# Tealdragon204/nightcore-to-flac-analyzer

Hardware: AMD Instinct MI355X
Metric: 10 s windows/sec (CQT+onset, 22.05 kHz mono) at 1/2/4/8 GPUs; % HBM roofline (higher is better)
Workload: dtype f32

## Files before the change

nightcore-to-flac-analyzer_amd/csrc/cqt.hip:

```cpp
#include <algorithm>

#include "nc_block.h"
#include "nc_decim.h"
#include "nc_engine.h"
#include "nc_piptrack.h"

namespace nc {


struct ChromaPlan {
  const float* sig;
  const int64_t* chunk_off;
  const int64_t* chunk_len;
  int n_chunks;
  int64_t* oct_off;
  int64_t* oct_len;
  int* n_frames;
  int* n_tframes;
  int64_t* tf_base;
};

__device__ __forceinline__ int64_t chunk_oct_floats(int64_t L) {
  int64_t acc = 0;
  for (int i = 1; i < 7; ++i) {
// ... 211 lines not shown
      for (int w = 1; w < D3_NT / 64; ++w) m = fmaxf(m, wmax[w]);
      xmax[c + (base == 0 ? oo3 : oct_off[c * 7 + 3]) / 256 + blockIdx.x] = m;
    }
    d3_level1_inplace(e0, o0, 4 * m0 - 72, L1, h, out1);
    __syncthreads();
    d3_level(e0, o0, D3_N2, 2 * m0 - 24, L2, h, e0 + D3_U2, o0 + D3_U2, out2, 24, 2 * D3_T);
    __syncthreads();
    d3_level(e0 + D3_U2, o0 + D3_U2, D3_T, m0, L3, h, nullptr, nullptr, out3, 0, D3_T);
  }
}

constexpr int TP_WAVES = 16;
#ifndef TP_DYN_
#define TP_DYN_ 1
#endif
using TpTw = StagedTw<1024>;

struct PeakArgs {
  const float* sig;
  const int64_t* chunk_off;
  const int64_t* chunk_len;
  const int* n_tframes;
  const int64_t* tf_base;
  const int64_t* tp_base;
  int n_chunks;
  int64_t total_tframes;
  const float2* tw;
  const float* hann2048;
  float* peak_pitch;
  float* peak_mag;
  int* chunk_npk;
  const int* tf_skip;
  unsigned long long* span = nullptr;
};

__global__ __launch_bounds__(TP_WAVES * 64) void tuning_peaks_kernel(PeakArgs a) {
  const Span span_(a.span);
  extern __shared__ __attribute__((aligned(16))) char smem[];
  float2* sh_tw = reinterpret_cast<float2*>(smem);
  const int lane0 = threadIdx.x & 63, wave = __builtin_amdgcn_readfirstlane(threadIdx.x >> 6);
  float2* sh_hann = sh_tw + ((TpTw::size + 1) & ~1);
  float2* fftbuf = sh_hann + 1024 + wave * LdsSize<1024>::value;
  __shared__ int sh_next;
  if (threadIdx.x == 0) sh_next = 0;
  fill_staged_tw<1024>(sh_tw, a.tw, threadIdx.x, TP_WAVES * 64);
  for (int i = threadIdx.x; i < 1024; i += TP_WAVES * 64) sh_hann[i] = reinterpret_cast<const float2*>(a.hann2048)[i];
  __syncthreads();
  float2 hw[16];
  lds_read16_strided<0, 64 * 8>(hw, lds_addr(sh_hann + fft_in_lane(lane0)));
  const int64_t n_groups = (a.total_tframes + TP_WAVES - 1) / TP_WAVES;
  const int64_t gb = n_groups * blockIdx.x / gridDim.x, ge = n_groups * (blockIdx.x + 1) / gridDim.x;
  const int64_t f0 = gb * TP_WAVES, f1 = std::min<int64_t>(ge * TP_WAVES, a.total_tframes);
  WgFrameQueue fq(&sh_next, lane0);
  int c = -1, nt = 0, skip = 0;
  int64_t cb = 0, ce = -1, coff = 0, clen = 0, ctf = 0;
  for (int64_t grp = gb; TP_DYN_ || grp < ge; ++grp) {
    const int64_t gf = TP_DYN_ ? f0 + fq.take(lane0) : grp * TP_WAVES + wave;
    if (gf >= (TP_DYN_ ? f1 : a.total_tframes)) break;
    if (gf >= ce) {
      if (c < 0) {
        int lo = 0, hi = a.n_chunks - 1;
        while (lo < hi) {
          const int mid = (lo + hi + 1) >> 1;
          if (a.tp_base[mid] <= gf) lo = mid;
// ... 5 lines not shown
        while (c + 1 < a.n_chunks && a.tp_base[c + 1] <= gf);
      }
      c = uniform32(c);
      cb = uniform64(a.tp_base[c]);
      ce = uniform64(c + 1 < a.n_chunks ? a.tp_base[c + 1] : INT64_MAX);
      skip = uniform32(a.tf_skip ? a.tf_skip[c] : 0);
      nt = uniform32(a.n_tframes[c]);
      coff = uniform64(a.chunk_off[c]);
      clen = uniform64(a.chunk_len[c]);
      ctf = uniform64(a.tf_base[c]);
    }
    const int t = (int)(gf - cb) + skip;
    if (t >= nt) continue;
    int lane = lane0;
    asm volatile("" : "+v"(lane));
    const int jin = fft_in_lane(lane);
    const int64_t off = coff;
    const float* x = a.sig + off;
    const int64_t L = clen;
    const int64_t s0 = (int64_t)t * 512 - 1024;
    FftIn<1024> in;
    if (s0 >= 0 && s0 + 2048 <= L) {
      float2 xv[16];
      if ((off & 1) == 0) {
        const float2* x2 = reinterpret_cast<const float2*>(x + s0);
#pragma unroll
        for (int r = 0; r < 16; ++r) xv[r] = x2[jin + 64 * r];
      } else {
        const float* xs = x + s0;
#pragma unroll
        for (int r = 0; r < 16; ++r) xv[r] = make_float2(xs[2 * (jin + 64 * r)], xs[2 * (jin + 64 * r) + 1]);
      }
#pragma unroll
      for (int r = 0; r < 16; ++r) in[0][r] = make_float2(xv[r].x * hw[r].x, xv[r].y * hw[r].y);
    } else {
// ... 13 lines not shown
    float* S = reinterpret_cast<float*>(fftbuf);
    float pmax = 0.0f;
    rsplit_mirror<TpTw::split, false>(v, sh_tw, lane, [&](int k, float2 X, float2 XN) {
      const float p1 = fmaf(X.x, X.x, X.y * X.y), p2 = fmaf(XN.x, XN.x, XN.y * XN.y);
      S[k] = p1;
      pmax = fmaxf(pmax, fmaxf(p1, p2));
    });
    const float mx = __fsqrt_rn(wave_max_u(pmax));
#pragma unroll
    for (int q = 0; q < (kPipHi - kPipLo + 3 + 63) / 64; ++q) {
      const int k = kPipLo - 1 + 64 * q + lane;
      if (64 * (q + 1) <= kPipHi - kPipLo + 3 || k <= kPipHi + 1) S[k] = __fsqrt_rn(S[k]);
    }
    piptrack_append([&](int k) { return S[k]; }, mx, lane, &a.chunk_npk[c], a.peak_pitch + ctf * kPeakSlots,
                    a.peak_mag + ctf * kPeakSlots, reinterpret_cast<int*>(S + kPipKpk));
  }
}

constexpr int TS_NT = 1024;
__device__ __forceinline__ int tuning_bin(float r) {
  const double rd = (double)r;
  int j = (int)floor((rd + 0.5) * 100.0);
  j = max(0, min(99, j));
  auto edge = [](int i) { return i == 100 ? 0.5 : (double)i * (1.0 / 100.0) + (-0.5); };
  while (j > 0 && rd < edge(j)) --j;
  while (j < 99 && rd >= edge(j + 1)) ++j;
  return j;
}

__device__ __forceinline__ unsigned fkey(float f) {
// ... 251 lines not shown
  const unsigned lg = xcd_remap(blockIdx.x + gridDim.x * blockIdx.y, gridDim.x * gridDim.y);
  const int bx = (int)(lg % gridDim.x);
  const int c = (int)(lg / gridDim.x);
  const int tid = threadIdx.x, lane = tid & 63;
  const int wave = __builtin_amdgcn_readfirstlane(tid >> 6);
  const int oct = CM_LO + wave;
  const int T = a.n_frames[c], ti = a.tuning_idx[c], ex = a.oct_ex[c * 7 + oct];
  const int64_t yoff = a.oct_off[c * 7 + oct], Ly = a.oct_len[c * 7 + oct];
  const int t0 = bx * CH_FR;
  if (t0 >= T) return;
  const int nfr = min(CH_FR, T - t0);
  const uint4* bsrc = a.bfrag + (size_t)ti * (CM_KS * CM_SLICE);
  auto fetch_slice = [&](int ks) {
#pragma unroll
    for (int q = 0; q < CM_GQ; ++q) {
      int i = wave + CM_NW * q;
      if (i >= CM_NT * 2) i = wave;
      cm_dma16(bsrc + ks * CM_SLICE + i * 64 + lane, sB + (ks % CM_R) * CM_SLICE + i * 64);
    }
  };
  fetch_slice(0);

  const float* y = a.ws_oct + yoff;
  const int hop = 512 >> oct;
  const float sx = ldexpf(1.0f, ex);
  const int64_t s0 = (int64_t)t0 * hop - 512;
  const int S = (CH_FR - 1) * hop + kCqtNfft;
  const bool vec = s0 >= 0 && s0 + S <= Ly && (reinterpret_cast<uintptr_t>(y) & 15) == 0;
  const int kq = 8 * (lane >> 4);

  constexpr int aoffs[8] = {cm_aoff(0), cm_aoff(1), cm_aoff(2), cm_aoff(3), cm_aoff(4), cm_aoff(5), cm_aoff(6), cm_aoff(7)};
  const int pad = cm_pad(oct);
  const int img = cm_img(oct);
// ... 663 lines not shown
  pa.sig = sig;
  pa.chunk_off = chunk_off;
  pa.chunk_len = chunk_len;
  pa.n_tframes = w.n_tframes;
  pa.tf_base = w.tf_base;
  pa.tp_base = tp_base;
  pa.tf_skip = tf_skip;
  pa.n_chunks = n;
  pa.total_tframes = tfr - tf_skip_total;
  pa.tw = ctx.t.tw;
  pa.hann2048 = ctx.t.hann2048;
  pa.peak_pitch = w.peak_pitch;
  pa.peak_mag = w.peak_mag;
  pa.chunk_npk = w.chunk_npk;
  {
    const size_t lds = (((TpTw::size + 1) & ~1) + 1024 + (size_t)TP_WAVES * LdsSize<1024>::value) * sizeof(float2);
    const int64_t groups = (pa.total_tframes + TP_WAVES - 1) / TP_WAVES;
    const int grid = (int)std::max<int64_t>(1, std::min<int64_t>(groups, ctx.chroma_cus > 0 ? ctx.chroma_cus : ctx.num_cu));
    {
      KTimer kt_(ctx, "tuning_peaks", st);
      pa.span = kt_.span();
      hipLaunchKernelGGL(tuning_peaks_kernel, dim3(grid), dim3(TP_WAVES * 64), lds, st, pa);
    }
  }
  if (wait_event) NC_HIP(hipStreamWaitEvent(st, static_cast<hipEvent_t>(wait_event), 0));
  {
    KTimer kt_(ctx, "tuning_select", st);
    OctScale os;
    os.xmax = w.xmax;
    os.oct_off = w.oct_off;
    os.oct_len = w.oct_len;
// ... 57 lines not shown
```

nightcore-to-flac-analyzer_amd/csrc/stft.hip:

```cpp
#include <algorithm>

#include "nc_block.h"
#include "nc_engine.h"
#include "nc_piptrack.h"

#include "stft_args.h"

namespace nc {

constexpr int SM_HANN2 = 1024;
constexpr int SM_WAVES = 16;
constexpr int SM_THREADS = SM_WAVES * 64;
constexpr int SM_HALF = 528;
constexpr size_t SM_LDS_RESERVE = 150 * 1024;
#ifndef SM_NOEN_
#define SM_NOEN_ 0
#endif
#ifndef SM_SYNC_
#define SM_SYNC_ 0
#endif
#ifndef SM_DYN_
#define SM_DYN_ 1
#endif
using SmTw = StagedTw<1024>;

constexpr int kMelJ0 = 3, kMelJ1 = 14;
constexpr int kMelJ0w = 4, kMelJ1w = 17;
constexpr int kMelB = 7;

template <int J>
__device__ __forceinline__ void mel_unrolled(const float* pw, const float4* w4, int lo, int nj, int lane, float& acc) {
#pragma unroll
  for (int j0 = 0; j0 < J; j0 += kMelB) {
    float4 p[kMelB], w[kMelB];
#pragma unroll
    for (int j = 0; j < kMelB; ++j)
      if (j0 + j < J) {
        p[j] = *reinterpret_cast<const float4*>(pw + lo + 4 * (j0 + j));
        w[j] = w4[(j0 + j) * 64 + lane];
// ... 13 lines not shown
  }
  return lo;
}

__host__ __device__ __forceinline__ int al4(int n) { return (n + 3) & ~3; }

constexpr int SM_MT = 128;
__host__ __device__ __forceinline__ int mel_pack(int lo4, int nj4, int band) { return lo4 | (nj4 << 11) | (band << 16); }

size_t stft_mel_lds_bytes(int mel_j) {
  return (size_t)al4(SmTw::size) * sizeof(float2) + (size_t)mel_j * 64 * sizeof(float4) +
         (size_t)SM_HANN2 * sizeof(float2) + (size_t)SM_MT * sizeof(int) +
         (size_t)SM_WAVES * SM_HALF * sizeof(float2);
}

__device__ __forceinline__ int sm_j1(int l) {
  const int G = l >> 4, i = l & 15;
  return 4 * (8 * (G >> 1) + (i >> 1)) + (i & 1) + 2 * (G & 1);
}
__device__ __forceinline__ int sm_j2(int l) {
  return (l & 7) + 8 * (l >> 5) + 16 * ((l & 31) >> 3);
}
__host__ __device__ constexpr int sm_boff(int b) { return b == 0 ? 0 : b == 1 ? 136 : b == 2 ? 264 : 400; }
constexpr int kPipKpkHalf = 512;
static_assert(kPipKpkHalf >= kPipHi - kPipLo + 3 && kPipKpkHalf + (kPipHi - kPipLo + 1) <= 2 * SM_HALF,
              "piptrack half-slot layout");

#define NC_W_(v, o) "ds_write_b64 %[wb], %[" #v "] offset:" #o "\n\t"
#define NC_R_(d, b, o) "ds_read_b64 %[" #d "], %[" #b "] offset:" #o "\n\t"

__device__ __forceinline__ void sm_exchange1(const float2 (&v)[16], float2 (&u)[16], uint32_t wb, uint32_t rb) {
  nc_f2v i0 = {v[0].x, v[0].y}, i1 = {v[1].x, v[1].y}, i2 = {v[2].x, v[2].y}, i3 = {v[3].x, v[3].y};
  nc_f2v i4 = {v[4].x, v[4].y}, i5 = {v[5].x, v[5].y}, i6 = {v[6].x, v[6].y}, i7 = {v[7].x, v[7].y};
  nc_f2v i8 = {v[8].x, v[8].y}, i9 = {v[9].x, v[9].y}, i10 = {v[10].x, v[10].y}, i11 = {v[11].x, v[11].y};
  nc_f2v i12 = {v[12].x, v[12].y}, i13 = {v[13].x, v[13].y}, i14 = {v[14].x, v[14].y}, i15 = {v[15].x, v[15].y};
  nc_f2v d0, d1, d2, d3, d4, d5, d6, d7, d8, d9, d10, d11, d12, d13, d14, d15;
  unsigned long long sv;
  asm volatile(
      NC_W_(i0, 0) NC_W_(i1, 8) NC_W_(i2, 16) NC_W_(i3, 24) NC_W_(i4, 32) NC_W_(i5, 40) NC_W_(i6, 48) NC_W_(i7, 56)
      "s_mov_b64 %[sv], exec\n\t"
      "s_mov_b32 exec_hi, 0\n\t"
      NC_R_(d0, rb, 0) NC_R_(d1, rb, 264) NC_R_(d2, rb, 528) NC_R_(d3, rb, 792) NC_R_(d4, rb, 1056)
      NC_R_(d5, rb, 1320) NC_R_(d6, rb, 1584) NC_R_(d7, rb, 1848) NC_R_(d8, rb, 2112) NC_R_(d9, rb, 2376)
      NC_R_(d10, rb, 2640) NC_R_(d11, rb, 2904) NC_R_(d12, rb, 3168) NC_R_(d13, rb, 3432) NC_R_(d14, rb, 3696)
      NC_R_(d15, rb, 3960)
      "s_mov_b64 exec, %[sv]\n\t"
      NC_W_(i8, 0) NC_W_(i9, 8) NC_W_(i10, 16) NC_W_(i11, 24) NC_W_(i12, 32) NC_W_(i13, 40) NC_W_(i14, 48)
      NC_W_(i15, 56)
      "s_mov_b32 exec_lo, 0\n\t"
      NC_R_(d0, rb, 0) NC_R_(d1, rb, 264) NC_R_(d2, rb, 528) NC_R_(d3, rb, 792) NC_R_(d4, rb, 1056)
      NC_R_(d5, rb, 1320) NC_R_(d6, rb, 1584) NC_R_(d7, rb, 1848) NC_R_(d8, rb, 2112) NC_R_(d9, rb, 2376)
      NC_R_(d10, rb, 2640) NC_R_(d11, rb, 2904) NC_R_(d12, rb, 3168) NC_R_(d13, rb, 3432) NC_R_(d14, rb, 3696)
      NC_R_(d15, rb, 3960)
      "s_mov_b64 exec, %[sv]\n\t"
      "s_waitcnt lgkmcnt(0)"
      : [d0] "=&v"(d0), [d1] "=&v"(d1), [d2] "=&v"(d2), [d3] "=&v"(d3), [d4] "=&v"(d4), [d5] "=&v"(d5),
        [d6] "=&v"(d6), [d7] "=&v"(d7), [d8] "=&v"(d8), [d9] "=&v"(d9), [d10] "=&v"(d10), [d11] "=&v"(d11),
        [d12] "=&v"(d12), [d13] "=&v"(d13), [d14] "=&v"(d14), [d15] "=&v"(d15), [sv] "=&s"(sv)
      : [wb] "v"(wb), [rb] "v"(rb), [i0] "v"(i0), [i1] "v"(i1), [i2] "v"(i2), [i3] "v"(i3), [i4] "v"(i4),
        [i5] "v"(i5), [i6] "v"(i6), [i7] "v"(i7), [i8] "v"(i8), [i9] "v"(i9), [i10] "v"(i10), [i11] "v"(i11),
        [i12] "v"(i12), [i13] "v"(i13), [i14] "v"(i14), [i15] "v"(i15)
      : "memory");
  const nc_f2v d[16] = {d0, d1, d2, d3, d4, d5, d6, d7, d8, d9, d10, d11, d12, d13, d14, d15};
#pragma unroll
  for (int r = 0; r < 16; ++r) u[r] = make_float2(d[r].x, d[r].y);
}

__device__ __forceinline__ void sm_exchange2(const float2 (&v)[16], float2 (&o)[16], uint32_t wb, uint32_t r0,
                                             uint32_t r1, uint32_t r2, uint32_t r3) {
  nc_f2v i0 = {v[0].x, v[0].y}, i1 = {v[1].x, v[1].y}, i2 = {v[2].x, v[2].y}, i3 = {v[3].x, v[3].y};
  nc_f2v i4 = {v[4].x, v[4].y}, i5 = {v[5].x, v[5].y}, i6 = {v[6].x, v[6].y}, i7 = {v[7].x, v[7].y};
  nc_f2v i8 = {v[8].x, v[8].y}, i9 = {v[9].x, v[9].y}, i10 = {v[10].x, v[10].y}, i11 = {v[11].x, v[11].y};
  nc_f2v i12 = {v[12].x, v[12].y}, i13 = {v[13].x, v[13].y}, i14 = {v[14].x, v[14].y}, i15 = {v[15].x, v[15].y};
  nc_f2v d0, d1, d2, d3, d4, d5, d6, d7, d8, d9, d10, d11, d12, d13, d14, d15;
  asm volatile(
      NC_W_(i0, 0) NC_W_(i1, 128) NC_W_(i2, 256) NC_W_(i3, 384) NC_W_(i4, 512) NC_W_(i5, 640) NC_W_(i6, 768)
      NC_W_(i7, 896)
      NC_R_(d0, r0, 0) NC_R_(d1, r0, 1088) NC_R_(d2, r0, 2112) NC_R_(d3, r0, 3200)
      NC_R_(d4, r1, 0) NC_R_(d5, r1, 1088) NC_R_(d6, r1, 2112) NC_R_(d7, r1, 3200)
      NC_W_(i8, 0) NC_W_(i9, 128) NC_W_(i10, 256) NC_W_(i11, 384) NC_W_(i12, 512) NC_W_(i13, 640) NC_W_(i14, 768)
      NC_W_(i15, 896)
      NC_R_(d8, r2, 0) NC_R_(d9, r2, 1088) NC_R_(d10, r2, 2112) NC_R_(d11, r2, 3200)
      NC_R_(d12, r3, 0) NC_R_(d13, r3, 1088) NC_R_(d14, r3, 2112) NC_R_(d15, r3, 3200)
      "s_waitcnt lgkmcnt(0)"
      : [d0] "=&v"(d0), [d1] "=&v"(d1), [d2] "=&v"(d2), [d3] "=&v"(d3), [d4] "=&v"(d4), [d5] "=&v"(d5),
        [d6] "=&v"(d6), [d7] "=&v"(d7), [d8] "=&v"(d8), [d9] "=&v"(d9), [d10] "=&v"(d10), [d11] "=&v"(d11),
        [d12] "=&v"(d12), [d13] "=&v"(d13), [d14] "=&v"(d14), [d15] "=&v"(d15)
      : [wb] "v"(wb), [r0] "v"(r0), [r1] "v"(r1), [r2] "v"(r2), [r3] "v"(r3), [i0] "v"(i0), [i1] "v"(i1),
        [i2] "v"(i2), [i3] "v"(i3), [i4] "v"(i4), [i5] "v"(i5), [i6] "v"(i6), [i7] "v"(i7), [i8] "v"(i8),
        [i9] "v"(i9), [i10] "v"(i10), [i11] "v"(i11), [i12] "v"(i12), [i13] "v"(i13), [i14] "v"(i14),
        [i15] "v"(i15)
      : "memory");
  const nc_f2v d[16] = {d0, d1, d2, d3, d4, d5, d6, d7, d8, d9, d10, d11, d12, d13, d14, d15};
#pragma unroll
  for (int r = 0; r < 16; ++r) o[r] = make_float2(d[r].x, d[r].y);
}
#undef NC_W_
#undef NC_R_

template <bool H512, bool EN, int J0 = kMelJ0, int J1 = kMelJ1>
__global__ __launch_bounds__(SM_THREADS) void stft_mel_kernel(StftMelArgs a) {
  const Span span_(a.span);
  extern __shared__ __attribute__((aligned(16))) char smem[];
  float2* sh_tw = reinterpret_cast<float2*>(smem);
  float4* sh_w4 = reinterpret_cast<float4*>(sh_tw + al4(SmTw::size));
  const int lane0 = threadIdx.x & 63, wave = __builtin_amdgcn_readfirstlane(threadIdx.x >> 6);
  float2* sh_hann = reinterpret_cast<float2*>(sh_w4 + (a.mel_j0 + a.mel_j1) * 64);
  int* sh_mt = reinterpret_cast<int*>(sh_hann + SM_HANN2);
  float2* slot = reinterpret_cast<float2*>(sh_mt + SM_MT) + wave * SM_HALF;

  __shared__ int sh_next;
  if (threadIdx.x == 0) sh_next = 0;
  fill_staged_tw<1024>(sh_tw, a.tw, threadIdx.x, SM_THREADS);
// ... 39 lines not shown
      t0 = uniform64(a.frame_base && a.seq_t0 ? a.seq_t0[s] : 0);
      act = !a.active || a.active[s];
      L = uniform64(a.seq_len ? a.seq_len[s] : a.uniform_len);
      off = uniform64(a.seq_off[s]);
      wc = uniform32(a.win_chunk ? a.win_chunk[s] : -1);
    }
    if (!act) continue;
    const int64_t t = g - sb + t0;
    const float* x = a.sig + off;
    const int64_t s0 = t * a.hop - 1024;

    int lane = lane0;
    asm volatile("" : "+v"(lane));
    const int jin = sm_j1(lane);
    const float2* twl = sh_tw;
    const float* hann = a.hann2048;
    float2 in[16];
    double e = 0.0;
    const bool interior = s0 >= 0 && s0 + 2048 <= L;
    if (interior) {
      float2 xv[16];
      if ((off & 1) == 0) {
        const float2* x2 = reinterpret_cast<const float2*>(x + s0);
#pragma unroll
        for (int r = 0; r < 16; ++r) xv[r] = x2[jin + 64 * r];
      } else {
        const float* xs = x + s0;
#pragma unroll
        for (int r = 0; r < 16; ++r) xv[r] = make_float2(xs[2 * (jin + 64 * r)], xs[2 * (jin + 64 * r) + 1]);
      }
#pragma unroll
      for (int r = 0; r < 16; ++r) {
        const int n = jin + 64 * r;
        const float2 v = xv[r];
        const float2 h = hw[r];
        if (EN && r >= 8 && r < 12) {
          const bool in_hop = H512 || 2 * n - 1024 < a.hop;
          const double dx = in_hop ? (double)v.x : 0.0, dy = in_hop ? (double)v.y : 0.0;
          e = fma(dx, dx, e);
          e = fma(dy, dy, e);
        }
        in[r] = make_float2(v.x * h.x, v.y * h.y);
      }
    } else {
#pragma unroll
      for (int r = 0; r < 16; ++r) {
        const int n = jin + 64 * r;
        const int64_t i0 = s0 + 2 * n;
        const float x0 = (i0 >= 0 && i0 < L) ? x[i0] : 0.0f;
        const float x1 = (i0 + 1 >= 0 && i0 + 1 < L) ? x[i0 + 1] : 0.0f;
        if (EN && r >= 8 && r < 12) {
          const int q = 2 * n - 1024;
          if (q < a.hop) {
            e = fma((double)x0, (double)x0, e);
            e = fma((double)x1, (double)x1, e);
          }
        }
        in[r] = make_float2(x0 * hann[2 * n], x1 * hann[2 * n + 1]);
      }
    }
    if (EN) {
      e = wave_sum_u(e);
      if (lane == 0) a.frame_energy[g] = e;
    }
    DFT<16>::run(in);
    const int j2 = sm_j2(lane), k2 = j2 & 15;
    float2 v2[16];
    sm_exchange1(in, v2, lds_addr(slot + 8 * jin + (jin >> 2)), lds_addr(slot + (lane & 31)));
    {
      const uint32_t ta = lds_addr(twl + k2);
      tw_batch3<0, 16 * 8>(v2 + 1, ta);
      tw_batch3<3, 16 * 8>(v2 + 4, ta);
      tw_batch3<6, 16 * 8>(v2 + 7, ta);
      tw_batch3<9, 16 * 8>(v2 + 10, ta);
      tw_batch3<12, 16 * 8>(v2 + 13, ta);
    }
    DFT<16>::run(v2);
    float2 v[4][4];
    {
      const int b2 = j2 >> 4;
      float2 o[16];
      sm_exchange2(v2, o, lds_addr(slot + sm_boff(b2) + k2), lds_addr(slot + mirror_J(lane, 0)),
                   lds_addr(slot + mirror_J(lane, 1)), lds_addr(slot + (mirror_J(lane, 2) - 128)),
                   lds_addr(slot + (mirror_J(lane, 3) - 128)));
      static_for<4>([&](auto bc) {
        constexpr int b = decltype(bc)::value;
        float2 w[3];
        const uint32_t ta = lds_addr(twl + SmTw::s3 + mirror_J(lane, b));
        lds_read3<0, 2048, 4096>(w, ta, ta, ta);
        v[b][0] = o[4 * b];
#pragma unroll
        for (int r = 1; r < 4; ++r) v[b][r] = cmul(o[4 * b + r], w[r - 1]);
        DFT<4>::run(v[b]);
      });
    }
    float* pw = reinterpret_cast<float*>(slot);
    const bool pip = wc >= 0 && t < a.tp_frames;
    float pmax = 0.0f;
    if (pip) {
      rsplit_mirror<SmTw::split, false>(v, twl, lane, [&](int k, float2 X, float2 XN) {
        const float p1 = fmaf(X.x, X.x, X.y * X.y), p2 = fmaf(XN.x, XN.x, XN.y * XN.y);
        pw[k] = p1;
        pw[1024 - k] = p2;
        pmax = fmaxf(pmax, fmaxf(p1, p2));
      });
    } else {
      rsplit_mirror<SmTw::split, false>(v, twl, lane, [&](int k, float2 X, float2 XN) {
        pw[k] = fmaf(X.x, X.x, X.y * X.y);
        pw[1024 - k] = fmaf(XN.x, XN.x, XN.y * XN.y);
      });
    }
    float acc0 = 0.0f, acc1 = 0.0f;
    const int mt0 = sh_mt[lane], mt1 = sh_mt[64 + lane];
    mel_unrolled<J0>(pw, mw4, mt0 & 2047, (mt0 >> 11) & 31, lane, acc0);
    mel_unrolled<J1>(pw, mw4 + J0 * 64, mt1 & 2047, (mt1 >> 11) & 31, lane, acc1);
    const float db0 = db10_floor(acc0);
    const float db1 = db10_floor(acc1);
    float* row = a.sdb + g * 128;
    row[mt0 >> 16] = db0;
    row[mt1 >> 16] = db1;
    const float mx = wave_max_u(fmaxf(db0, db1));
    if (lane == 0) a.frame_max[g] = mx;
    if (pip) {
      const float pm = __fsqrt_rn(wave_max_u(pmax));
      constexpr int kPipQ = (kPipHi - kPipLo + 3 + 63) / 64;
      float pv[kPipQ];
#pragma unroll
      for (int q = 0; q < kPipQ; ++q) {
        const int k = kPipLo - 1 + 64 * q + lane;
        pv[q] = (64 * (q + 1) <= kPipHi - kPipLo + 3 || k <= kPipHi + 1) ? pw[k] : 0.0f;
      }
      asm volatile("" ::: "memory");
#pragma unroll
      for (int q = 0; q < kPipQ; ++q) {
        const int k = kPipLo - 1 + 64 * q + lane;
        if (64 * (q + 1) <= kPipHi - kPipLo + 3 || k <= kPipHi + 1) pw[k - (kPipLo - 1)] = __fsqrt_rn(pv[q]);
      }
      const int64_t base = uniform64(a.chunk_tf_base[wc]) * kPeakSlots;
      piptrack_append([&](int k) { return pw[k - (kPipLo - 1)]; }, pm, lane, &a.chunk_npk[wc], a.peak_pitch + base,
                      a.peak_mag + base, reinterpret_cast<int*>(pw + kPipKpkHalf));
    }
  }
}

int launch_stft_mel(Context& ctx, const StftMelArgs& args, hipStream_t st) {
  if (args.total_frames <= 0) return 0;
  StftMelArgs a = args;
  a.tw = ctx.t.tw;
  a.hann2048 = ctx.t.hann2048;
  a.mel_lo = ctx.t.mel_lo;
  a.mel_len = ctx.t.mel_len;
  a.mel_off = ctx.t.mel_off;
  a.mel_w = ctx.t.mel_w;
  a.mel_nnz = ctx.t.mel_nnz;
  a.mel_w4 = ctx.t.mel_w4;
// ... 58 lines not shown
```

Baseline: 486,600.

## Share the STFT frame FFT core with the tuning-peaks kernel and use compact LDS slots

Moves the hand-scheduled 1024-point frame FFT (custom lane mapping, inline-asm LDS exchanges, power and piptrack helpers) out of the STFT kernel into a shared header. The tuning-peaks kernel now uses this path by default in place of its generic Stockham FFT, with a smaller per-wave LDS slot, while still reserving the old LDS size. The chroma B-fragment prefetch also skips redundant duplicate DMA loads for waves past the slice count. The aim is fewer LDS operations and less FFT instruction overhead in the tuning kernel. The piptrack layout is now half-slot, and behaviour changes if the compact layout or the new lane mapping differ subtly from the old path.

```diff
diff --git a/nightcore-to-flac-analyzer_amd/csrc/cqt.hip b/nightcore-to-flac-analyzer_amd/csrc/cqt.hip
--- a/nightcore-to-flac-analyzer_amd/csrc/cqt.hip
+++ b/nightcore-to-flac-analyzer_amd/csrc/cqt.hip
@@ -3,7 +3,7 @@
 #include "nc_block.h"
 #include "nc_decim.h"
 #include "nc_engine.h"
-#include "nc_piptrack.h"
+#include "nc_frame_fft.h"
 
 namespace nc {
 
@@ -249,7 +249,15 @@
 #ifndef TP_DYN_
 #define TP_DYN_ 1
 #endif
-using TpTw = StagedTw<1024>;
+#ifndef TP_CORE_
+#define TP_CORE_ 1
+#endif
+using TpTw = FrameTw;
+constexpr int TP_SLOT = TP_CORE_ ? SM_HALF : LdsSize<1024>::value;
+constexpr size_t TP_LDS_BYTES = (((TpTw::size + 1) & ~1) + 1024 + (size_t)TP_WAVES * TP_SLOT) * sizeof(float2);
+#ifndef TP_LDS_RESERVE_
+#define TP_LDS_RESERVE_ ((((TpTw::size + 1) & ~1) + 1024 + TP_WAVES * LdsSize<1024>::value) * 8)
+#endif
 
 struct PeakArgs {
   const float* sig;
@@ -275,14 +283,14 @@
   float2* sh_tw = reinterpret_cast<float2*>(smem);
   const int lane0 = threadIdx.x & 63, wave = __builtin_amdgcn_readfirstlane(threadIdx.x >> 6);
   float2* sh_hann = sh_tw + ((TpTw::size + 1) & ~1);
-  float2* fftbuf = sh_hann + 1024 + wave * LdsSize<1024>::value;
+  float2* fftbuf = sh_hann + 1024 + wave * TP_SLOT;
   __shared__ int sh_next;
   if (threadIdx.x == 0) sh_next = 0;
   fill_staged_tw<1024>(sh_tw, a.tw, threadIdx.x, TP_WAVES * 64);
   for (int i = threadIdx.x; i < 1024; i += TP_WAVES * 64) sh_hann[i] = reinterpret_cast<const float2*>(a.hann2048)[i];
   __syncthreads();
   float2 hw[16];
-  lds_read16_strided<0, 64 * 8>(hw, lds_addr(sh_hann + fft_in_lane(lane0)));
+  lds_read16_strided<0, 64 * 8>(hw, lds_addr(sh_hann + (TP_CORE_ ? sm_j1(lane0) : fft_in_lane(lane0))));
   const int64_t n_groups = (a.total_tframes + TP_WAVES - 1) / TP_WAVES;
   const int64_t gb = n_groups * blockIdx.x / gridDim.x, ge = n_groups * (blockIdx.x + 1) / gridDim.x;
   const int64_t f0 = gb * TP_WAVES, f1 = std::min<int64_t>(ge * TP_WAVES, a.total_tframes);
@@ -318,11 +326,22 @@
     if (t >= nt) continue;
     int lane = lane0;
     asm volatile("" : "+v"(lane));
-    const int jin = fft_in_lane(lane);
+    const int jin = TP_CORE_ ? sm_j1(lane) : fft_in_lane(lane);
     const int64_t off = coff;
     const float* x = a.sig + off;
     const int64_t L = clen;
     const int64_t s0 = (int64_t)t * 512 - 1024;
+#if TP_CORE_
+    float2 in[16];
+    double e_ = 0.0;
+    frame_load_hann<false, true>(x, s0, L, (off & 1) != 0, 512, jin, hw, a.hann2048, in, e_);
+    float2 v[4][4];
+    frame_fft1024(in, fftbuf, sh_tw, lane, jin, v);
+    float* pw = reinterpret_cast<float*>(fftbuf);
+    float pmax = 0.0f;
+    frame_power<true, false>(v, sh_tw, lane, pw, pmax);
+    frame_piptrack(pw, pmax, lane, &a.chunk_npk[c], a.peak_pitch + ctf * kPeakSlots, a.peak_mag + ctf * kPeakSlots);
+#else
     FftIn<1024> in;
     if (s0 >= 0 && s0 + 2048 <= L) {
       float2 xv[16];
@@ -366,6 +385,7 @@
     }
     piptrack_append([&](int k) { return S[k]; }, mx, lane, &a.chunk_npk[c], a.peak_pitch + ctf * kPeakSlots,
                     a.peak_mag + ctf * kPeakSlots, reinterpret_cast<int*>(S + kPipKpk));
+#endif
   }
 }
 
@@ -647,9 +667,8 @@
   auto fetch_slice = [&](int ks) {
 #pragma unroll
     for (int q = 0; q < CM_GQ; ++q) {
-      int i = wave + CM_NW * q;
-      if (i >= CM_NT * 2) i = wave;
-      cm_dma16(bsrc + ks * CM_SLICE + i * 64 + lane, sB + (ks % CM_R) * CM_SLICE + i * 64);
+      const int i = wave + CM_NW * q;
+      if (i < CM_NT * 2) cm_dma16(bsrc + ks * CM_SLICE + i * 64 + lane, sB + (ks % CM_R) * CM_SLICE + i * 64);
     }
   };
   fetch_slice(0);
@@ -1343,7 +1362,7 @@
   pa.peak_mag = w.peak_mag;
   pa.chunk_npk = w.chunk_npk;
   {
-    const size_t lds = (((TpTw::size + 1) & ~1) + 1024 + (size_t)TP_WAVES * LdsSize<1024>::value) * sizeof(float2);
+    const size_t lds = std::max<size_t>(TP_LDS_BYTES, TP_LDS_RESERVE_);
     const int64_t groups = (pa.total_tframes + TP_WAVES - 1) / TP_WAVES;
     const int grid = (int)std::max<int64_t>(1, std::min<int64_t>(groups, ctx.chroma_cus > 0 ? ctx.chroma_cus : ctx.num_cu));
     {
diff --git a/nightcore-to-flac-analyzer_amd/csrc/nc_frame_fft.h b/nightcore-to-flac-analyzer_amd/csrc/nc_frame_fft.h
--- /dev/null
+++ b/nightcore-to-flac-analyzer_amd/csrc/nc_frame_fft.h
@@ -0,0 +1,204 @@
+#pragma once
+#include "nc_device.h"
+#include "nc_piptrack.h"
+
+namespace nc {
+
+using FrameTw = StagedTw<1024>;
+constexpr int SM_HALF = 528;
+
+__device__ __forceinline__ int sm_j1(int l) {
+  const int G = l >> 4, i = l & 15;
+  return 4 * (8 * (G >> 1) + (i >> 1)) + (i & 1) + 2 * (G & 1);
+}
+__device__ __forceinline__ int sm_j2(int l) {
+  return (l & 7) + 8 * (l >> 5) + 16 * ((l & 31) >> 3);
+}
+__host__ __device__ constexpr int sm_boff(int b) { return b == 0 ? 0 : b == 1 ? 136 : b == 2 ? 264 : 400; }
+constexpr int kPipKpkHalf = 512;
+static_assert(kPipKpkHalf >= kPipHi - kPipLo + 3 && kPipKpkHalf + (kPipHi - kPipLo + 1) <= 2 * SM_HALF,
+              "piptrack half-slot layout");
+
+#define NC_W_(v, o) "ds_write_b64 %[wb], %[" #v "] offset:" #o "\n\t"
+#define NC_R_(d, b, o) "ds_read_b64 %[" #d "], %[" #b "] offset:" #o "\n\t"
+
+__device__ __forceinline__ void sm_exchange1(const float2 (&v)[16], float2 (&u)[16], uint32_t wb, uint32_t rb) {
+  nc_f2v i0 = {v[0].x, v[0].y}, i1 = {v[1].x, v[1].y}, i2 = {v[2].x, v[2].y}, i3 = {v[3].x, v[3].y};
+  nc_f2v i4 = {v[4].x, v[4].y}, i5 = {v[5].x, v[5].y}, i6 = {v[6].x, v[6].y}, i7 = {v[7].x, v[7].y};
+  nc_f2v i8 = {v[8].x, v[8].y}, i9 = {v[9].x, v[9].y}, i10 = {v[10].x, v[10].y}, i11 = {v[11].x, v[11].y};
+  nc_f2v i12 = {v[12].x, v[12].y}, i13 = {v[13].x, v[13].y}, i14 = {v[14].x, v[14].y}, i15 = {v[15].x, v[15].y};
+  nc_f2v d0, d1, d2, d3, d4, d5, d6, d7, d8, d9, d10, d11, d12, d13, d14, d15;
+  unsigned long long sv;
+  asm volatile(
+      NC_W_(i0, 0) NC_W_(i1, 8) NC_W_(i2, 16) NC_W_(i3, 24) NC_W_(i4, 32) NC_W_(i5, 40) NC_W_(i6, 48) NC_W_(i7, 56)
+      "s_mov_b64 %[sv], exec\n\t"
+      "s_mov_b32 exec_hi, 0\n\t"
+      NC_R_(d0, rb, 0) NC_R_(d1, rb, 264) NC_R_(d2, rb, 528) NC_R_(d3, rb, 792) NC_R_(d4, rb, 1056)
+      NC_R_(d5, rb, 1320) NC_R_(d6, rb, 1584) NC_R_(d7, rb, 1848) NC_R_(d8, rb, 2112) NC_R_(d9, rb, 2376)
+      NC_R_(d10, rb, 2640) NC_R_(d11, rb, 2904) NC_R_(d12, rb, 3168) NC_R_(d13, rb, 3432) NC_R_(d14, rb, 3696)
+      NC_R_(d15, rb, 3960)
+      "s_mov_b64 exec, %[sv]\n\t"
+      NC_W_(i8, 0) NC_W_(i9, 8) NC_W_(i10, 16) NC_W_(i11, 24) NC_W_(i12, 32) NC_W_(i13, 40) NC_W_(i14, 48)
+      NC_W_(i15, 56)
+      "s_mov_b32 exec_lo, 0\n\t"
+      NC_R_(d0, rb, 0) NC_R_(d1, rb, 264) NC_R_(d2, rb, 528) NC_R_(d3, rb, 792) NC_R_(d4, rb, 1056)
+      NC_R_(d5, rb, 1320) NC_R_(d6, rb, 1584) NC_R_(d7, rb, 1848) NC_R_(d8, rb, 2112) NC_R_(d9, rb, 2376)
+      NC_R_(d10, rb, 2640) NC_R_(d11, rb, 2904) NC_R_(d12, rb, 3168) NC_R_(d13, rb, 3432) NC_R_(d14, rb, 3696)
+      NC_R_(d15, rb, 3960)
+      "s_mov_b64 exec, %[sv]\n\t"
+      "s_waitcnt lgkmcnt(0)"
+      : [d0] "=&v"(d0), [d1] "=&v"(d1), [d2] "=&v"(d2), [d3] "=&v"(d3), [d4] "=&v"(d4), [d5] "=&v"(d5),
+        [d6] "=&v"(d6), [d7] "=&v"(d7), [d8] "=&v"(d8), [d9] "=&v"(d9), [d10] "=&v"(d10), [d11] "=&v"(d11),
+        [d12] "=&v"(d12), [d13] "=&v"(d13), [d14] "=&v"(d14), [d15] "=&v"(d15), [sv] "=&s"(sv)
+      : [wb] "v"(wb), [rb] "v"(rb), [i0] "v"(i0), [i1] "v"(i1), [i2] "v"(i2), [i3] "v"(i3), [i4] "v"(i4),
+        [i5] "v"(i5), [i6] "v"(i6), [i7] "v"(i7), [i8] "v"(i8), [i9] "v"(i9), [i10] "v"(i10), [i11] "v"(i11),
+        [i12] "v"(i12), [i13] "v"(i13), [i14] "v"(i14), [i15] "v"(i15)
+      : "memory");
+  const nc_f2v d[16] = {d0, d1, d2, d3, d4, d5, d6, d7, d8, d9, d10, d11, d12, d13, d14, d15};
+#pragma unroll
+  for (int r = 0; r < 16; ++r) u[r] = make_float2(d[r].x, d[r].y);
+}
+
+__device__ __forceinline__ void sm_exchange2(const float2 (&v)[16], float2 (&o)[16], uint32_t wb, uint32_t r0,
+                                             uint32_t r1, uint32_t r2, uint32_t r3) {
+  nc_f2v i0 = {v[0].x, v[0].y}, i1 = {v[1].x, v[1].y}, i2 = {v[2].x, v[2].y}, i3 = {v[3].x, v[3].y};
+  nc_f2v i4 = {v[4].x, v[4].y}, i5 = {v[5].x, v[5].y}, i6 = {v[6].x, v[6].y}, i7 = {v[7].x, v[7].y};
+  nc_f2v i8 = {v[8].x, v[8].y}, i9 = {v[9].x, v[9].y}, i10 = {v[10].x, v[10].y}, i11 = {v[11].x, v[11].y};
+  nc_f2v i12 = {v[12].x, v[12].y}, i13 = {v[13].x, v[13].y}, i14 = {v[14].x, v[14].y}, i15 = {v[15].x, v[15].y};
+  nc_f2v d0, d1, d2, d3, d4, d5, d6, d7, d8, d9, d10, d11, d12, d13, d14, d15;
+  asm volatile(
+      NC_W_(i0, 0) NC_W_(i1, 128) NC_W_(i2, 256) NC_W_(i3, 384) NC_W_(i4, 512) NC_W_(i5, 640) NC_W_(i6, 768)
+      NC_W_(i7, 896)
+      NC_R_(d0, r0, 0) NC_R_(d1, r0, 1088) NC_R_(d2, r0, 2112) NC_R_(d3, r0, 3200)
+      NC_R_(d4, r1, 0) NC_R_(d5, r1, 1088) NC_R_(d6, r1, 2112) NC_R_(d7, r1, 3200)
+      NC_W_(i8, 0) NC_W_(i9, 128) NC_W_(i10, 256) NC_W_(i11, 384) NC_W_(i12, 512) NC_W_(i13, 640) NC_W_(i14, 768)
+      NC_W_(i15, 896)
+      NC_R_(d8, r2, 0) NC_R_(d9, r2, 1088) NC_R_(d10, r2, 2112) NC_R_(d11, r2, 3200)
+      NC_R_(d12, r3, 0) NC_R_(d13, r3, 1088) NC_R_(d14, r3, 2112) NC_R_(d15, r3, 3200)
+      "s_waitcnt lgkmcnt(0)"
+      : [d0] "=&v"(d0), [d1] "=&v"(d1), [d2] "=&v"(d2), [d3] "=&v"(d3), [d4] "=&v"(d4), [d5] "=&v"(d5),
+        [d6] "=&v"(d6), [d7] "=&v"(d7), [d8] "=&v"(d8), [d9] "=&v"(d9), [d10] "=&v"(d10), [d11] "=&v"(d11),
+        [d12] "=&v"(d12), [d13] "=&v"(d13), [d14] "=&v"(d14), [d15] "=&v"(d15)
+      : [wb] "v"(wb), [r0] "v"(r0), [r1] "v"(r1), [r2] "v"(r2), [r3] "v"(r3), [i0] "v"(i0), [i1] "v"(i1),
+        [i2] "v"(i2), [i3] "v"(i3), [i4] "v"(i4), [i5] "v"(i5), [i6] "v"(i6), [i7] "v"(i7), [i8] "v"(i8),
+        [i9] "v"(i9), [i10] "v"(i10), [i11] "v"(i11), [i12] "v"(i12), [i13] "v"(i13), [i14] "v"(i14),
+        [i15] "v"(i15)
+      : "memory");
+  const nc_f2v d[16] = {d0, d1, d2, d3, d4, d5, d6, d7, d8, d9, d10, d11, d12, d13, d14, d15};
+#pragma unroll
+  for (int r = 0; r < 16; ++r) o[r] = make_float2(d[r].x, d[r].y);
+}
+#undef NC_W_
+#undef NC_R_
+
+template <bool EN, bool H512>
+__device__ __forceinline__ void frame_load_hann(const float* x, int64_t s0, int64_t L, bool odd, int hop, int jin,
+                                                const float2 (&hw)[16], const float* hann, float2 (&in)[16],
+                                                double& e) {
+  const bool interior = s0 >= 0 && s0 + 2048 <= L;
+  if (interior) {
+    float2 xv[16];
+    if (!odd) {
+      const float2* x2 = reinterpret_cast<const float2*>(x + s0);
+#pragma unroll
+      for (int r = 0; r < 16; ++r) xv[r] = x2[jin + 64 * r];
+    } else {
+      const float* xs = x + s0;
+#pragma unroll
+      for (int r = 0; r < 16; ++r) xv[r] = make_float2(xs[2 * (jin + 64 * r)], xs[2 * (jin + 64 * r) + 1]);
+    }
+#pragma unroll
+    for (int r = 0; r < 16; ++r) {
+      const int n = jin + 64 * r;
+      const float2 v = xv[r];
+      const float2 h = hw[r];
+      if (EN && r >= 8 && r < 12) {
+        const bool in_hop = H512 || 2 * n - 1024 < hop;
+        const double dx = in_hop ? (double)v.x : 0.0, dy = in_hop ? (double)v.y : 0.0;
+        e = fma(dx, dx, e);
+        e = fma(dy, dy, e);
+      }
+      in[r] = make_float2(v.x * h.x, v.y * h.y);
+    }
+  } else {
+#pragma unroll
+    for (int r = 0; r < 16; ++r) {
+      const int n = jin + 64 * r;
+      const int64_t i0 = s0 + 2 * n;
+      const float x0 = (i0 >= 0 && i0 < L) ? x[i0] : 0.0f;
+      const float x1 = (i0 + 1 >= 0 && i0 + 1 < L) ? x[i0 + 1] : 0.0f;
+      if (EN && r >= 8 && r < 12) {
+        const int q = 2 * n - 1024;
+        if (q < hop) {
+          e = fma((double)x0, (double)x0, e);
+          e = fma((double)x1, (double)x1, e);
+        }
+      }
+      in[r] = make_float2(x0 * hann[2 * n], x1 * hann[2 * n + 1]);
+    }
+  }
+}
+
+__device__ __forceinline__ void frame_fft1024(float2 (&in)[16], float2* slot, const float2* twl, int lane, int jin,
+                                              float2 (&v)[4][4]) {
+  DFT<16>::run(in);
+  const int j2 = sm_j2(lane), k2 = j2 & 15;
+  float2 v2[16];
+  sm_exchange1(in, v2, lds_addr(slot + 8 * jin + (jin >> 2)), lds_addr(slot + (lane & 31)));
+  {
+    const uint32_t ta = lds_addr(twl + k2);
+    tw_batch3<0, 16 * 8>(v2 + 1, ta);
+    tw_batch3<3, 16 * 8>(v2 + 4, ta);
+    tw_batch3<6, 16 * 8>(v2 + 7, ta);
+    tw_batch3<9, 16 * 8>(v2 + 10, ta);
+    tw_batch3<12, 16 * 8>(v2 + 13, ta);
+  }
+  DFT<16>::run(v2);
+  const int b2 = j2 >> 4;
+  float2 o[16];
+  sm_exchange2(v2, o, lds_addr(slot + sm_boff(b2) + k2), lds_addr(slot + mirror_J(lane, 0)),
+               lds_addr(slot + mirror_J(lane, 1)), lds_addr(slot + (mirror_J(lane, 2) - 128)),
+               lds_addr(slot + (mirror_J(lane, 3) - 128)));
+  static_for<4>([&](auto bc) {
+    constexpr int b = decltype(bc)::value;
+    float2 w[3];
+    const uint32_t ta = lds_addr(twl + FrameTw::s3 + mirror_J(lane, b));
+    lds_read3<0, 2048, 4096>(w, ta, ta, ta);
+    v[b][0] = o[4 * b];
+#pragma unroll
+    for (int r = 1; r < 4; ++r) v[b][r] = cmul(o[4 * b + r], w[r - 1]);
+    DFT<4>::run(v[b]);
+  });
+}
+
+template <bool PMAX, bool HI>
+__device__ __forceinline__ void frame_power(const float2 (&v)[4][4], const float2* twl, int lane, float* pw,
+                                            float& pmax) {
+  rsplit_mirror<FrameTw::split, false>(v, twl, lane, [&](int k, float2 X, float2 XN) {
+    const float p1 = fmaf(X.x, X.x, X.y * X.y), p2 = fmaf(XN.x, XN.x, XN.y * XN.y);
+    pw[k] = p1;
+    if (HI) pw[1024 - k] = p2;
+    if (PMAX) pmax = fmaxf(pmax, fmaxf(p1, p2));
+  });
+}
+
+__device__ __forceinline__ void frame_piptrack(float* pw, float pmax, int lane, int* npk, float* pp, float* pm_out) {
+  const float pm = __fsqrt_rn(wave_max_u(pmax));
+  constexpr int kPipQ = (kPipHi - kPipLo + 3 + 63) / 64;
+  float pv[kPipQ];
+#pragma unroll
+  for (int q = 0; q < kPipQ; ++q) {
+    const int k = kPipLo - 1 + 64 * q + lane;
+    pv[q] = (64 * (q + 1) <= kPipHi - kPipLo + 3 || k <= kPipHi + 1) ? pw[k] : 0.0f;
+  }
+  asm volatile("" ::: "memory");
+#pragma unroll
+  for (int q = 0; q < kPipQ; ++q) {
+    const int k = kPipLo - 1 + 64 * q + lane;
+    if (64 * (q + 1) <= kPipHi - kPipLo + 3 || k <= kPipHi + 1) pw[k - (kPipLo - 1)] = __fsqrt_rn(pv[q]);
+  }
+  piptrack_append([&](int k) { return pw[k - (kPipLo - 1)]; }, pm, lane, npk, pp, pm_out,
+                  reinterpret_cast<int*>(pw + kPipKpkHalf));
+}
+
+}
diff --git a/nightcore-to-flac-analyzer_amd/csrc/stft.hip b/nightcore-to-flac-analyzer_amd/csrc/stft.hip
--- a/nightcore-to-flac-analyzer_amd/csrc/stft.hip
+++ b/nightcore-to-flac-analyzer_amd/csrc/stft.hip
@@ -2,7 +2,7 @@
 
 #include "nc_block.h"
 #include "nc_engine.h"
-#include "nc_piptrack.h"
+#include "nc_frame_fft.h"
 
 #include "stft_args.h"
 
@@ -11,7 +11,6 @@
 constexpr int SM_HANN2 = 1024;
 constexpr int SM_WAVES = 16;
 constexpr int SM_THREADS = SM_WAVES * 64;
-constexpr int SM_HALF = 528;
 constexpr size_t SM_LDS_RESERVE = 150 * 1024;
 #ifndef SM_NOEN_
 #define SM_NOEN_ 0
@@ -22,7 +21,7 @@
 #ifndef SM_DYN_
 #define SM_DYN_ 1
 #endif
-using SmTw = StagedTw<1024>;
+using SmTw = FrameTw;
 
 constexpr int kMelJ0 = 3, kMelJ1 = 14;
 constexpr int kMelJ0w = 4, kMelJ1w = 17;
@@ -66,89 +65,6 @@
          (size_t)SM_WAVES * SM_HALF * sizeof(float2);
 }
 
-__device__ __forceinline__ int sm_j1(int l) {
-  const int G = l >> 4, i = l & 15;
-  return 4 * (8 * (G >> 1) + (i >> 1)) + (i & 1) + 2 * (G & 1);
-}
-__device__ __forceinline__ int sm_j2(int l) {
-  return (l & 7) + 8 * (l >> 5) + 16 * ((l & 31) >> 3);
-}
-__host__ __device__ constexpr int sm_boff(int b) { return b == 0 ? 0 : b == 1 ? 136 : b == 2 ? 264 : 400; }
-constexpr int kPipKpkHalf = 512;
-static_assert(kPipKpkHalf >= kPipHi - kPipLo + 3 && kPipKpkHalf + (kPipHi - kPipLo + 1) <= 2 * SM_HALF,
-              "piptrack half-slot layout");
-
-#define NC_W_(v, o) "ds_write_b64 %[wb], %[" #v "] offset:" #o "\n\t"
-#define NC_R_(d, b, o) "ds_read_b64 %[" #d "], %[" #b "] offset:" #o "\n\t"
-
-__device__ __forceinline__ void sm_exchange1(const float2 (&v)[16], float2 (&u)[16], uint32_t wb, uint32_t rb) {
-  nc_f2v i0 = {v[0].x, v[0].y}, i1 = {v[1].x, v[1].y}, i2 = {v[2].x, v[2].y}, i3 = {v[3].x, v[3].y};
-  nc_f2v i4 = {v[4].x, v[4].y}, i5 = {v[5].x, v[5].y}, i6 = {v[6].x, v[6].y}, i7 = {v[7].x, v[7].y};
-  nc_f2v i8 = {v[8].x, v[8].y}, i9 = {v[9].x, v[9].y}, i10 = {v[10].x, v[10].y}, i11 = {v[11].x, v[11].y};
-  nc_f2v i12 = {v[12].x, v[12].y}, i13 = {v[13].x, v[13].y}, i14 = {v[14].x, v[14].y}, i15 = {v[15].x, v[15].y};
-  nc_f2v d0, d1, d2, d3, d4, d5, d6, d7, d8, d9, d10, d11, d12, d13, d14, d15;
-  unsigned long long sv;
-  asm volatile(
-      NC_W_(i0, 0) NC_W_(i1, 8) NC_W_(i2, 16) NC_W_(i3, 24) NC_W_(i4, 32) NC_W_(i5, 40) NC_W_(i6, 48) NC_W_(i7, 56)
-      "s_mov_b64 %[sv], exec\n\t"
-      "s_mov_b32 exec_hi, 0\n\t"
-      NC_R_(d0, rb, 0) NC_R_(d1, rb, 264) NC_R_(d2, rb, 528) NC_R_(d3, rb, 792) NC_R_(d4, rb, 1056)
-      NC_R_(d5, rb, 1320) NC_R_(d6, rb, 1584) NC_R_(d7, rb, 1848) NC_R_(d8, rb, 2112) NC_R_(d9, rb, 2376)
-      NC_R_(d10, rb, 2640) NC_R_(d11, rb, 2904) NC_R_(d12, rb, 3168) NC_R_(d13, rb, 3432) NC_R_(d14, rb, 3696)
-      NC_R_(d15, rb, 3960)
-      "s_mov_b64 exec, %[sv]\n\t"
-      NC_W_(i8, 0) NC_W_(i9, 8) NC_W_(i10, 16) NC_W_(i11, 24) NC_W_(i12, 32) NC_W_(i13, 40) NC_W_(i14, 48)
-      NC_W_(i15, 56)
-      "s_mov_b32 exec_lo, 0\n\t"
-      NC_R_(d0, rb, 0) NC_R_(d1, rb, 264) NC_R_(d2, rb, 528) NC_R_(d3, rb, 792) NC_R_(d4, rb, 1056)
-      NC_R_(d5, rb, 1320) NC_R_(d6, rb, 1584) NC_R_(d7, rb, 1848) NC_R_(d8, rb, 2112) NC_R_(d9, rb, 2376)
-      NC_R_(d10, rb, 2640) NC_R_(d11, rb, 2904) NC_R_(d12, rb, 3168) NC_R_(d13, rb, 3432) NC_R_(d14, rb, 3696)
-      NC_R_(d15, rb, 3960)
-      "s_mov_b64 exec, %[sv]\n\t"
-      "s_waitcnt lgkmcnt(0)"
-      : [d0] "=&v"(d0), [d1] "=&v"(d1), [d2] "=&v"(d2), [d3] "=&v"(d3), [d4] "=&v"(d4), [d5] "=&v"(d5),
-        [d6] "=&v"(d6), [d7] "=&v"(d7), [d8] "=&v"(d8), [d9] "=&v"(d9), [d10] "=&v"(d10), [d11] "=&v"(d11),
-        [d12] "=&v"(d12), [d13] "=&v"(d13), [d14] "=&v"(d14), [d15] "=&v"(d15), [sv] "=&s"(sv)
-      : [wb] "v"(wb), [rb] "v"(rb), [i0] "v"(i0), [i1] "v"(i1), [i2] "v"(i2), [i3] "v"(i3), [i4] "v"(i4),
-        [i5] "v"(i5), [i6] "v"(i6), [i7] "v"(i7), [i8] "v"(i8), [i9] "v"(i9), [i10] "v"(i10), [i11] "v"(i11),
-        [i12] "v"(i12), [i13] "v"(i13), [i14] "v"(i14), [i15] "v"(i15)
-      : "memory");
-  const nc_f2v d[16] = {d0, d1, d2, d3, d4, d5, d6, d7, d8, d9, d10, d11, d12, d13, d14, d15};
-#pragma unroll
-  for (int r = 0; r < 16; ++r) u[r] = make_float2(d[r].x, d[r].y);
-}
-
-__device__ __forceinline__ void sm_exchange2(const float2 (&v)[16], float2 (&o)[16], uint32_t wb, uint32_t r0,
-                                             uint32_t r1, uint32_t r2, uint32_t r3) {
-  nc_f2v i0 = {v[0].x, v[0].y}, i1 = {v[1].x, v[1].y}, i2 = {v[2].x, v[2].y}, i3 = {v[3].x, v[3].y};
-  nc_f2v i4 = {v[4].x, v[4].y}, i5 = {v[5].x, v[5].y}, i6 = {v[6].x, v[6].y}, i7 = {v[7].x, v[7].y};
-  nc_f2v i8 = {v[8].x, v[8].y}, i9 = {v[9].x, v[9].y}, i10 = {v[10].x, v[10].y}, i11 = {v[11].x, v[11].y};
-  nc_f2v i12 = {v[12].x, v[12].y}, i13 = {v[13].x, v[13].y}, i14 = {v[14].x, v[14].y}, i15 = {v[15].x, v[15].y};
-  nc_f2v d0, d1, d2, d3, d4, d5, d6, d7, d8, d9, d10, d11, d12, d13, d14, d15;
-  asm volatile(
-      NC_W_(i0, 0) NC_W_(i1, 128) NC_W_(i2, 256) NC_W_(i3, 384) NC_W_(i4, 512) NC_W_(i5, 640) NC_W_(i6, 768)
-      NC_W_(i7, 896)
-      NC_R_(d0, r0, 0) NC_R_(d1, r0, 1088) NC_R_(d2, r0, 2112) NC_R_(d3, r0, 3200)
-      NC_R_(d4, r1, 0) NC_R_(d5, r1, 1088) NC_R_(d6, r1, 2112) NC_R_(d7, r1, 3200)
-      NC_W_(i8, 0) NC_W_(i9, 128) NC_W_(i10, 256) NC_W_(i11, 384) NC_W_(i12, 512) NC_W_(i13, 640) NC_W_(i14, 768)
-      NC_W_(i15, 896)
-      NC_R_(d8, r2, 0) NC_R_(d9, r2, 1088) NC_R_(d10, r2, 2112) NC_R_(d11, r2, 3200)
-      NC_R_(d12, r3, 0) NC_R_(d13, r3, 1088) NC_R_(d14, r3, 2112) NC_R_(d15, r3, 3200)
-      "s_waitcnt lgkmcnt(0)"
-      : [d0] "=&v"(d0), [d1] "=&v"(d1), [d2] "=&v"(d2), [d3] "=&v"(d3), [d4] "=&v"(d4), [d5] "=&v"(d5),
-        [d6] "=&v"(d6), [d7] "=&v"(d7), [d8] "=&v"(d8), [d9] "=&v"(d9), [d10] "=&v"(d10), [d11] "=&v"(d11),
-        [d12] "=&v"(d12), [d13] "=&v"(d13), [d14] "=&v"(d14), [d15] "=&v"(d15)
-      : [wb] "v"(wb), [r0] "v"(r0), [r1] "v"(r1), [r2] "v"(r2), [r3] "v"(r3), [i0] "v"(i0), [i1] "v"(i1),
-        [i2] "v"(i2), [i3] "v"(i3), [i4] "v"(i4), [i5] "v"(i5), [i6] "v"(i6), [i7] "v"(i7), [i8] "v"(i8),
-        [i9] "v"(i9), [i10] "v"(i10), [i11] "v"(i11), [i12] "v"(i12), [i13] "v"(i13), [i14] "v"(i14),
-        [i15] "v"(i15)
-      : "memory");
-  const nc_f2v d[16] = {d0, d1, d2, d3, d4, d5, d6, d7, d8, d9, d10, d11, d12, d13, d14, d15};
-#pragma unroll
-  for (int r = 0; r < 16; ++r) o[r] = make_float2(d[r].x, d[r].y);
-}
-#undef NC_W_
-#undef NC_R_
 
 template <bool H512, bool EN, int J0 = kMelJ0, int J1 = kMelJ1>
 __global__ __launch_bounds__(SM_THREADS) void stft_mel_kernel(StftMelArgs a) {
@@ -218,102 +134,20 @@
     asm volatile("" : "+v"(lane));
     const int jin = sm_j1(lane);
     const float2* twl = sh_tw;
-    const float* hann = a.hann2048;
     float2 in[16];
     double e = 0.0;
-    const bool interior = s0 >= 0 && s0 + 2048 <= L;
-    if (interior) {
-      float2 xv[16];
-      if ((off & 1) == 0) {
-        const float2* x2 = reinterpret_cast<const float2*>(x + s0);
-#pragma unroll
-        for (int r = 0; r < 16; ++r) xv[r] = x2[jin + 64 * r];
-      } else {
-        const float* xs = x + s0;
-#pragma unroll
-        for (int r = 0; r < 16; ++r) xv[r] = make_float2(xs[2 * (jin + 64 * r)], xs[2 * (jin + 64 * r) + 1]);
-      }
-#pragma unroll
-      for (int r = 0; r < 16; ++r) {
-        const int n = jin + 64 * r;
-        const float2 v = xv[r];
-        const float2 h = hw[r];
-        if (EN && r >= 8 && r < 12) {
-          const bool in_hop = H512 || 2 * n - 1024 < a.hop;
-          const double dx = in_hop ? (double)v.x : 0.0, dy = in_hop ? (double)v.y : 0.0;
-          e = fma(dx, dx, e);
-          e = fma(dy, dy, e);
-        }
-        in[r] = make_float2(v.x * h.x, v.y * h.y);
-      }
-    } else {
-#pragma unroll
-      for (int r = 0; r < 16; ++r) {
-        const int n = jin + 64 * r;
-        const int64_t i0 = s0 + 2 * n;
-        const float x0 = (i0 >= 0 && i0 < L) ? x[i0] : 0.0f;
-        const float x1 = (i0 + 1 >= 0 && i0 + 1 < L) ? x[i0 + 1] : 0.0f;
-        if (EN && r >= 8 && r < 12) {
-          const int q = 2 * n - 1024;
-          if (q < a.hop) {
-            e = fma((double)x0, (double)x0, e);
-            e = fma((double)x1, (double)x1, e);
-          }
-        }
-        in[r] = make_float2(x0 * hann[2 * n], x1 * hann[2 * n + 1]);
-      }
-    }
+    frame_load_hann<EN, H512>(x, s0, L, (off & 1) != 0, a.hop, jin, hw, a.hann2048, in, e);
     if (EN) {
       e = wave_sum_u(e);
       if (lane == 0) a.frame_energy[g] = e;
     }
-    DFT<16>::run(in);
-    const int j2 = sm_j2(lane), k2 = j2 & 15;
-    float2 v2[16];
-    sm_exchange1(in, v2, lds_addr(slot + 8 * jin + (jin >> 2)), lds_addr(slot + (lane & 31)));
-    {
-      const uint32_t ta = lds_addr(twl + k2);
-      tw_batch3<0, 16 * 8>(v2 + 1, ta);
-      tw_batch3<3, 16 * 8>(v2 + 4, ta);
-      tw_batch3<6, 16 * 8>(v2 + 7, ta);
-      tw_batch3<9, 16 * 8>(v2 + 10, ta);
-      tw_batch3<12, 16 * 8>(v2 + 13, ta);
-    }
-    DFT<16>::run(v2);
     float2 v[4][4];
-    {
-      const int b2 = j2 >> 4;
-      float2 o[16];
-      sm_exchange2(v2, o, lds_addr(slot + sm_boff(b2) + k2), lds_addr(slot + mirror_J(lane, 0)),
-                   lds_addr(slot + mirror_J(lane, 1)), lds_addr(slot + (mirror_J(lane, 2) - 128)),
-                   lds_addr(slot + (mirror_J(lane, 3) - 128)));
-      static_for<4>([&](auto bc) {
-        constexpr int b = decltype(bc)::value;
-        float2 w[3];
-        const uint32_t ta = lds_addr(twl + SmTw::s3 + mirror_J(lane, b));
-        lds_read3<0, 2048, 4096>(w, ta, ta, ta);
-        v[b][0] = o[4 * b];
-#pragma unroll
-        for (int r = 1; r < 4; ++r) v[b][r] = cmul(o[4 * b + r], w[r - 1]);
-        DFT<4>::run(v[b]);
-      });
-    }
+    frame_fft1024(in, slot, twl, lane, jin, v);
     float* pw = reinterpret_cast<float*>(slot);
     const bool pip = wc >= 0 && t < a.tp_frames;
     float pmax = 0.0f;
-    if (pip) {
-      rsplit_mirror<SmTw::split, false>(v, twl, lane, [&](int k, float2 X, float2 XN) {
-        const float p1 = fmaf(X.x, X.x, X.y * X.y), p2 = fmaf(XN.x, XN.x, XN.y * XN.y);
-        pw[k] = p1;
-        pw[1024 - k] = p2;
-        pmax = fmaxf(pmax, fmaxf(p1, p2));
-      });
-    } else {
-      rsplit_mirror<SmTw::split, false>(v, twl, lane, [&](int k, float2 X, float2 XN) {
-        pw[k] = fmaf(X.x, X.x, X.y * X.y);
-        pw[1024 - k] = fmaf(XN.x, XN.x, XN.y * XN.y);
-      });
-    }
+    if (pip) frame_power<true, true>(v, twl, lane, pw, pmax);
+    else frame_power<false, true>(v, twl, lane, pw, pmax);
     float acc0 = 0.0f, acc1 = 0.0f;
     const int mt0 = sh_mt[lane], mt1 = sh_mt[64 + lane];
     mel_unrolled<J0>(pw, mw4, mt0 & 2047, (mt0 >> 11) & 31, lane, acc0);
@@ -326,23 +160,8 @@
     const float mx = wave_max_u(fmaxf(db0, db1));
     if (lane == 0) a.frame_max[g] = mx;
     if (pip) {
-      const float pm = __fsqrt_rn(wave_max_u(pmax));
-      constexpr int kPipQ = (kPipHi - kPipLo + 3 + 63) / 64;
-      float pv[kPipQ];
-#pragma unroll
-      for (int q = 0; q < kPipQ; ++q) {
-        const int k = kPipLo - 1 + 64 * q + lane;
-        pv[q] = (64 * (q + 1) <= kPipHi - kPipLo + 3 || k <= kPipHi + 1) ? pw[k] : 0.0f;
-      }
-      asm volatile("" ::: "memory");
-#pragma unroll
-      for (int q = 0; q < kPipQ; ++q) {
-        const int k = kPipLo - 1 + 64 * q + lane;
-        if (64 * (q + 1) <= kPipHi - kPipLo + 3 || k <= kPipHi + 1) pw[k - (kPipLo - 1)] = __fsqrt_rn(pv[q]);
-      }
       const int64_t base = uniform64(a.chunk_tf_base[wc]) * kPeakSlots;
-      piptrack_append([&](int k) { return pw[k - (kPipLo - 1)]; }, pm, lane, &a.chunk_npk[wc], a.peak_pitch + base,
-                      a.peak_mag + base, reinterpret_cast<int*>(pw + kPipKpkHalf));
+      frame_piptrack(pw, pmax, lane, &a.chunk_npk[wc], a.peak_pitch + base, a.peak_mag + base);
     }
   }
 }
```

Measured after the change: 478,300. 0.983x the previous value.
